# kcat/openal-soft

Hardware: NVIDIA H100
Metric: voice-samples/s mixed (HRTF, bsinc24, 1024-frame updates) (higher is better)
Workload: dtype f32

## Files before the change

openal-soft_b200/csrc/async_ptx.cuh:

```cuda
#pragma once
#include <cstdint>
#include <cuda_runtime.h>

namespace b200mix {

__device__ __forceinline__ uint32_t smem_u32(const void *p)
{ return static_cast<uint32_t>(__cvta_generic_to_shared(p)); }

__device__ __forceinline__ void mbar_init(uint64_t *bar, uint32_t count)
{ asm volatile("mbarrier.init.shared::cta.b64 [%0], %1;" :: "r"(smem_u32(bar)), "r"(count) : "memory"); }
__device__ __forceinline__ void mbar_fence_init()
{ asm volatile("fence.mbarrier_init.release.cluster;" ::: "memory"); }
__device__ __forceinline__ void mbar_expect_tx(uint64_t *bar, uint32_t bytes)
{ asm volatile("mbarrier.arrive.expect_tx.shared::cta.b64 _, [%0], %1;" :: "r"(smem_u32(bar)), "r"(bytes) : "memory"); }
__device__ __forceinline__ void mbar_arrive(uint64_t *bar)
{ asm volatile("mbarrier.arrive.shared::cta.b64 _, [%0];" :: "r"(smem_u32(bar)) : "memory"); }
__device__ __forceinline__ bool mbar_try_wait(uint64_t *bar, uint32_t parity)
{
    uint32_t ok;
    asm volatile("{\n\t.reg .pred p;\n\t"
                 "mbarrier.try_wait.parity.shared::cta.b64 p, [%1], %2;\n\t"
                 "selp.u32 %0, 1, 0, p;\n\t}"
                 : "=r"(ok) : "r"(smem_u32(bar)), "r"(parity) : "memory");
    return ok != 0u;
}
__device__ __forceinline__ void mbar_wait(uint64_t *bar, uint32_t parity)
{ while(!mbar_try_wait(bar, parity)) { } }

__device__ __forceinline__ void bulk_g2s(void *dst_smem, const void *src_gmem, uint32_t bytes, uint64_t *bar)
{
    asm volatile("cp.async.bulk.shared::cluster.global.mbarrier::complete_tx::bytes [%0], [%1], %2, [%3];"
        :: "r"(smem_u32(dst_smem)), "l"(src_gmem), "r"(bytes), "r"(smem_u32(bar)) : "memory");
}
__device__ __forceinline__ void fence_proxy_async_smem()
{ asm volatile("fence.proxy.async.shared::cta;" ::: "memory"); }

__device__ __forceinline__ uint64_t wgmma_smem_desc(uint32_t saddr, uint32_t lbo_bytes, uint32_t sbo_bytes)
{
    return uint64_t((saddr >> 4) & 0x3fffu) | (uint64_t((lbo_bytes >> 4) & 0x3fffu) << 16)
        | (uint64_t((sbo_bytes >> 4) & 0x3fffu) << 32);
}
__device__ __forceinline__ void wgmma_fence() { asm volatile("wgmma.fence.sync.aligned;" ::: "memory"); }
__device__ __forceinline__ void wgmma_commit() { asm volatile("wgmma.commit_group.sync.aligned;" ::: "memory"); }
template<int N> __device__ __forceinline__ void wgmma_wait()
{ asm volatile("wgmma.wait_group.sync.aligned %0;" :: "n"(N) : "memory"); }
__device__ __forceinline__ void wgmma_m64n16k8_tf32(float (&d)[8], uint64_t adesc, uint64_t bdesc, bool accumulate)
{
    asm volatile("{\n\t.reg .pred p;\n\tsetp.ne.b32 p, %10, 0;\n\t"
                 "wgmma.mma_async.sync.aligned.m64n16k8.f32.tf32.tf32 "
                 "{%0,%1,%2,%3,%4,%5,%6,%7}, %8, %9, p, 1, 1;\n\t}"
        : "+f"(d[0]), "+f"(d[1]), "+f"(d[2]), "+f"(d[3]), "+f"(d[4]), "+f"(d[5]), "+f"(d[6]), "+f"(d[7])
        : "l"(adesc), "l"(bdesc), "r"(uint32_t(accumulate)) : "memory");
}

}
```

openal-soft_b200/csrc/b200mix.cu:

```cuda
#include "../../include/b200mix.h"

#include <algorithm>
#include <cmath>
#include <cstdio>
#include <cstdlib>
#include <cstring>
#include <new>
#include <string>
#include <vector>

#include <cuda_runtime.h>

#include <dlfcn.h>

#include "mixer_kernels.cuh"
#include "effect_kernels.cuh"
#include "shard_kernels.cuh"
#include "panmix_tc.cuh"
#include "param_kernels.hpp"
#include "efx_kernels.hpp"
#include "resampler_tables.hpp"
#include "hrtf_store.hpp"
#include "adpcm.hpp"

// ... 119 lines not shown
    bool reverb_upmix{false};
    bool mid_render{false}; uint32_t mid_frames{0};
    bool real_overwrite{false};
    std::vector<uint8_t> h_hrtf;
    std::vector<SendEntry> h_dry_entries;
    SendEntry *d_dry_entries{nullptr};
    uint32_t *d_dry_slot_start{nullptr};
    uint32_t num_dry_entries{0};
    bool dry_entries_dirty{true};
    float *d_dry_partial{nullptr};
    float *d_dry_geff{nullptr};
    float *d_send_geff{nullptr};
    float4 *d_dry_gramp{nullptr}, *d_send_gramp{nullptr};
    float *d_send_partial{nullptr};
    uint32_t send_partial_chunks{0}, max_slot_entries{0};
    bool profile{false};
    cudaEvent_t ev_mix0{nullptr}, ev_mix1{nullptr};
    bool ev_valid{false};
    static constexpr int kStages = 8;
    cudaEvent_t ev_stage[kStages + 1]{};
    bool stage_valid{false}; int profile_level{0};

    std::vector<uint8_t> h_active;
    std::vector<uint32_t> h_cost;
    std::vector<uint32_t> h_order;
    uint32_t *d_order{nullptr};
    uint32_t num_order{0};
    bool order_dirty{true};

    char *h_src{nullptr}, *d_src{nullptr}; uint32_t src_cap{0};
    cudaEvent_t src_done{nullptr}; bool src_busy{false};
    bool dev_filters{false};
    bool panmix_tc{false};

    struct Shard {
        uint32_t rank{0}, world{1}; int transport{0};
        char *own{nullptr}; size_t bytes{0};
        char *peer[kShardMaxWorld]{};
        size_t off_real{0}, off_wet{0}, real_floats{0}, wet_src_floats{0};
        uint32_t owned_max{0};
        uint32_t epoch{0};
        uint32_t *d_counters{nullptr};
        uint32_t *h_status{nullptr};
        cudaEvent_t ev[4]{};
        bool ev_wet{false}, ev_real{false};
        void *nccl_lib{nullptr}; void *comm{nullptr};
        int (*reduce)(const void*, void*, size_t, int, int, int, void*, cudaStream_t){nullptr};
        int (*allreduce)(const void*, void*, size_t, int, int, void*, cudaStream_t){nullptr};
        int (*comm_destroy)(void*){nullptr};
    } shard;

    uint32_t ir_pad{0};
    uint32_t voice_hi{0};
    void (*mix_fn)(const MixParams){nullptr};
    size_t mix_smem{0}; int mix_cdr{0}; int mix_blocks_per_sm{1};
    uint32_t reverb_seq{0};
    uint32_t *d_claim{nullptr};
    int fir_blocks_per_sm{0};
};

namespace {

#define CUDA_TRY(dev, expr) do { cudaError_t e_ = (expr); if(e_ != cudaSuccess) {            \
    (dev)->error = std::string(#expr) + ": " + cudaGetErrorString(e_); return B200MIX_ERR_CUDA; } } while(0)

template<typename T>
int dev_alloc(b200mix_device *d, T *&p, size_t count, bool zero = true)
{
    p = nullptr;
    if(count == 0) return B200MIX_OK;
    CUDA_TRY(d, cudaMalloc(reinterpret_cast<void**>(&p), count*sizeof(T)));
    if(zero) CUDA_TRY(d, cudaMemsetAsync(p, 0, count*sizeof(T), d->stream));
    return B200MIX_OK;
}

using MixKernel = void(*)(const MixParams);

struct FirVariant { MixKernel fn; size_t smem; };
FirVariant get_fir(uint32_t ir_size)
{
    if(ir_size <= 64u)
        return FirVariant{k_hrtf_fir<17, 64>, sizeof(FirSmem<kFirGS, 17, 64>)*kFirGroups};
    return FirVariant{k_hrtf_fir<19, 128>, sizeof(FirSmem<kFirGS, 19, 128>)*kFirGroups};
}

constexpr uint32_t kDryChunksMax = 128;

int ensure_dry_park(b200mix_device *d)
{
    const b200mix_device_desc &dd = d->desc;
    if(d->d_dry_entries) return B200MIX_OK;
    if(!d->d_xscratch)
        if(int rc = dev_alloc(d, d->d_xscratch, size_t(dd.max_voices)*kLine)) return rc;
    if(!d->d_sendinfo)
        if(int rc = dev_alloc(d, d->d_sendinfo, dd.max_voices)) return rc;
    if(int rc = dev_alloc(d, d->d_dry_entries, dd.max_voices)) return rc;
    if(dd.dry_channels > 4u && dd.dry_channels <= uint32_t(kPmN))
    {
        CUDA_TRY(d, cudaFuncSetAttribute(k_panmix_tc, cudaFuncAttributeMaxDynamicSharedMemorySize,
            kPmStages*kPmStageBytes + 1024));
        const char *simt = std::getenv("B200MIX_PANMIX_SIMT");
        d->panmix_tc = !(simt && simt[0] == '1');
    }
    if(int rc = dev_alloc(d, d->d_dry_slot_start, 2)) return rc;
    if(int rc = dev_alloc(d, d->d_dry_partial, size_t(kDryChunksMax)*dd.dry_channels*kLine)) return rc;
    if(int rc = dev_alloc(d, d->d_dry_geff, size_t(dd.max_voices)*dd.dry_channels)) return rc;
    if(int rc = dev_alloc(d, d->d_dry_gramp, size_t(dd.max_voices)*dd.dry_channels)) return rc;
    return B200MIX_OK;
}

static size_t align16(size_t v) { return (v + 15u) & ~size_t(15); }

int ensure_stage(b200mix_device *d, uint32_t n)
{
    if(n <= d->stage_cap) return B200MIX_OK;
    const b200mix_device_desc &dd = d->desc;
    if(d->stage_cap)
    {
        cudaStreamSynchronize(d->stream);
        cudaFreeHost(d->h_arena); cudaFree(d->d_arena);
        d->h_arena = nullptr; d->d_arena = nullptr;
    }
    const uint32_t cap = std::max<uint32_t>(n, 256u);
    const size_t bytes = align16(size_t(cap)*sizeof(VoiceUpdate))
        + align16(size_t(cap)*std::max<size_t>(size_t(dd.ir_size)*2, 4)*sizeof(float))
        + align16(size_t(cap)*dd.dry_channels*sizeof(float))
        + align16(size_t(cap)*dd.num_sends*dd.wet_channels*sizeof(float)) + 64;
    CUDA_TRY(d, cudaMallocHost(reinterpret_cast<void**>(&d->h_arena), bytes));
    CUDA_TRY(d, cudaMalloc(reinterpret_cast<void**>(&d->d_arena), bytes));
    d->h_upd = reinterpret_cast<VoiceUpdate*>(d->h_arena);
    d->stage_cap = cap;
    return B200MIX_OK;
}

const BsincTable *bsinc_for(const b200mix_device *d, uint32_t resampler)
{
    if(resampler < B200MIX_RESAMPLER_FAST_BSINC12 || resampler > B200MIX_RESAMPLER_BSINC48)
        return nullptr;
    return &d->bsinc[(resampler - B200MIX_RESAMPLER_FAST_BSINC12) >> 1];
}

}

extern "C" {

static void shard_release(b200mix_device *d);
static int ensure_filters(b200mix_device *d);

uint32_t b200mix_version(void) { return (1u<<16) | 1u; }

const char *b200mix_last_error(const b200mix_device *dev)
{ return dev ? dev->error.c_str() : g_create_error.c_str(); }

int b200mix_create(const b200mix_device_desc *desc, b200mix_device **out)
{
    if(!desc || !out || desc->struct_size != sizeof(b200mix_device_desc))
    { g_create_error = "bad descriptor"; return B200MIX_ERR_INVALID; }
    if(desc->dry_channels > B200MIX_MAX_DRY_CHANNELS || desc->wet_channels > B200MIX_MAX_WET_CHANNELS
        || desc->num_sends > B200MIX_MAX_SENDS || desc->ir_size > B200MIX_HRIR_LENGTH
        || desc->real_channels > B200MIX_MAX_DRY_CHANNELS || desc->max_voices == 0)
    { g_create_error = "descriptor out of range"; return B200MIX_ERR_INVALID; }
    if((desc->post_process == B200MIX_POST_UHJ && desc->dry_channels < 3)
        || (desc->post_process == B200MIX_POST_TSME && desc->dry_channels < 4))
    { g_create_error = "UHJ post-process needs W,X,Y dry channels"; return B200MIX_ERR_INVALID; }
    if((desc->post_process == B200MIX_POST_HRTF || desc->post_process == B200MIX_POST_UHJ
        || desc->post_process == B200MIX_POST_TSME)
// ... 1365 lines not shown
        std::stable_sort(d->h_order.begin(), d->h_order.end(),
            [d](uint32_t a, uint32_t b) { return d->h_cost[a] > d->h_cost[b]; });
        d->num_order = uint32_t(d->h_order.size());
        if(d->num_order)
        {
            CUDA_TRY(d, cudaMemcpyAsync(d->d_order, d->h_order.data(), d->num_order*sizeof(uint32_t),
                cudaMemcpyHostToDevice, d->stream));
            CUDA_TRY(d, cudaStreamSynchronize(d->stream));
        }
        d->order_dirty = false;
        d->order2_dirty = true;
        d->dry_entries_dirty = true;
    }
    if(d->d_filt && d->order2_dirty)
    {
        d->h_order2.clear();
        for(uint32_t v : d->h_order) if(d->dev_filters || d->h_dfilt[v]) d->h_order2.push_back(v);
        d->num_order2 = uint32_t(d->h_order2.size());
        if(d->num_order2)
        {
            CUDA_TRY(d, cudaMemcpyAsync(d->d_order2, d->h_order2.data(), d->num_order2*sizeof(uint32_t),
                cudaMemcpyHostToDevice, d->stream));
            CUDA_TRY(d, cudaStreamSynchronize(d->stream));
        }
        d->order2_dirty = false;
    }
    const bool hrtfDev = dd.ir_size > 0;
    const uint32_t nv = std::max(d->voice_hi, 1u);
    const uint32_t maxBlocks = uint32_t(d->num_sms*d->mix_blocks_per_sm);
    const uint32_t blocks = std::max(1u, std::min(maxBlocks, (d->num_order + kMixGroups - 1)/kMixGroups));

    MixParams P{};
    P.voices = d->d_voices; P.buffers = d->d_buffers;
    P.hrtf_tgt = d->d_hrtf_tgt; P.hrtf_old = d->d_hrtf_old;
    P.dry_cur = d->d_dry_cur; P.dry_tgt = d->d_dry_tgt;
    P.partial = d->d_partial;
    P.results = want_results ? d->d_results : nullptr;
    for(int i = 0;i < 3;++i) P.bsinc_tab[i] = d->d_bsinc[i];
    for(int i = 0;i < 2;++i) P.cubic_tab[i] = d->d_cubic[i];
    P.max_voices = nv; P.frames = frames; P.ir_pad = d->ir_pad;
    P.cd = dd.dry_channels; P.num_sends = dd.num_sends;
    P.order = d->d_order; P.num_order = d->num_order;
    P.xscratch = d->d_xscratch; P.sendinfo = d->d_sendinfo;
    P.filt = d->d_filt; P.filt_paths = 1u + dd.num_sends;
    P.qhdr = d->d_qhdr; P.queue = d->d_queue;
    P.claim = d->d_claim;
    P.dline = d->d_dline;
    stage_mark(d, 1);
    if(d->profile) cudaEventRecord(d->ev_mix0, d->stream);
    d->mix_fn<<<blocks, kMixGS*kMixGroups, d->mix_smem, d->stream>>>(P);
    ++d->launches;
    CUDA_TRY(d, cudaGetLastError());

    stage_mark(d, 2);
    size_t rows2 = 0;
    if(d->d_filt && d->num_order2)
    {
        FilterRunParams FP{};
        FP.filt = d->d_filt; FP.filt_paths = 1u + dd.num_sends; FP.sendinfo = d->d_sendinfo;
        FP.direct_order = d->d_order2; FP.num_direct = d->num_order2;
        FP.xscratch = d->d_xscratch; FP.dline = d->d_dline; FP.frames = frames;
        k_filters<<<(d->num_order2 + 31u)/32u, 32, 0, d->stream>>>(FP);
        ++d->launches;
        if(d->mix_cdr > 0)
        {
            const uint32_t blocks2 = std::max(1u, std::min(maxBlocks, (d->num_order2 + kMixGroups - 1)/kMixGroups));
            rows2 = blocks2;
            MixParams P2 = P;
            P2.order = d->d_order2; P2.num_order = d->num_order2;
            P2.partial = d->d_partial + d->partial_floats;
            P2.results = nullptr;
            k_mix_deferred<kMixGS, kMixGroups, 4><<<blocks2, kMixGS*kMixGroups,
                sizeof(DeferredSmem<kMixGroups, 4>), d->stream>>>(P2);
            ++d->launches;
        }
        CUDA_TRY(d, cudaGetLastError());
    }
    uint32_t firBlocks = 0;
    if(hrtfDev)
    {
        const FirVariant fir = get_fir(dd.ir_size);
        firBlocks = std::max(1u, std::min(uint32_t(d->num_sms*d->fir_blocks_per_sm),
            (d->num_order + kFirGroups - 1)/kFirGroups));
        fir.fn<<<firBlocks, kFirGS*kFirGroups, fir.smem, d->stream>>>(P);
        ++d->launches;
        CUDA_TRY(d, cudaGetLastError());
    }
    if(d->profile) { cudaEventRecord(d->ev_mix1, d->stream); d->ev_valid = true; }

    stage_mark(d, 3);
    if(hrtfDev)
    {
        const uint32_t len = 2*kAccumLen;
        k_reduce_rows<<<(len/4 + kReduceCols - 1)/kReduceCols, 1024, 0, d->stream>>>(d->d_partial, firBlocks, len,
            d->d_accum_sum, 0);
        ++d->launches;
    }
    if(d->mix_cdr > 0)
    {
        const uint32_t len = uint32_t(d->mix_cdr)*kLine;
        k_reduce_rows<<<(len/4 + kReduceCols - 1)/kReduceCols, 1024, 0, d->stream>>>(d->d_partial, blocks, len, d->d_dry, 1);
        ++d->launches;
        if(rows2)
        {
            k_reduce_rows<<<(len/4 + kReduceCols - 1)/kReduceCols, 1024, 0, d->stream>>>(d->d_partial + d->partial_floats,
                uint32_t(rows2), len, d->d_dry, 1);
            ++d->launches;
        }
    }
    CUDA_TRY(d, cudaGetLastError());

    stage_mark(d, 4);
    if(d->mix_cdr == 0 && d->d_dry_entries)
    {
        if(d->dry_entries_dirty)
        {
            d->h_dry_entries.clear();
            for(uint32_t v = 0;v < d->voice_hi;++v)
                if(d->h_active[v] && !d->h_hrtf[v]) d->h_dry_entries.push_back(SendEntry{v, 0u});
            d->num_dry_entries = uint32_t(d->h_dry_entries.size());
            const uint32_t ss[2] = {0u, d->num_dry_entries};
            CUDA_TRY(d, cudaMemcpyAsync(d->d_dry_slot_start, ss, sizeof(ss), cudaMemcpyHostToDevice, d->stream));
            if(d->num_dry_entries)
                CUDA_TRY(d, cudaMemcpyAsync(d->d_dry_entries, d->h_dry_entries.data(),
                    d->num_dry_entries*sizeof(SendEntry), cudaMemcpyHostToDevice, d->stream));
            CUDA_TRY(d, cudaStreamSynchronize(d->stream));
            d->dry_entries_dirty = false;
        }
        if(d->num_dry_entries)
        {
            SendMixParams DM{};
            DM.slot_start = d->d_dry_slot_start; DM.entries = d->d_dry_entries; DM.sendinfo = d->d_sendinfo;
            DM.xscratch = d->d_xscratch; DM.send_cur = d->d_dry_cur; DM.send_tgt = d->d_dry_tgt;
            DM.wet = d->d_dry; DM.frames = frames; DM.cw = dd.dry_channels; DM.num_sends = 1;
            DM.valid_bit = kSiDry; DM.dline = d->d_dline ? d->d_dline : d->d_xscratch;
            const uint32_t chunks = std::max(1u, std::min(kDryChunksMax, (d->num_dry_entries + 63u)/64u));
            DM.chunks = chunks; DM.partial = d->d_dry_partial; DM.geff = d->d_dry_geff; DM.gramp = d->d_dry_gramp;
            const bool tc = d->panmix_tc && dd.dry_channels > 4u && dd.dry_channels <= uint32_t(kPmN)
                && frames == uint32_t(kLine) && chunks > 1u;
            if(int rc = run_bus_mix(d, DM, d->num_dry_entries, 1u, tc)) return rc;
        }
    }

    stage_mark(d, 5);
    if((d->active_slots || force_sends) && d->d_wet && d->d_slot_start)
    {
        if(d->sends_dirty)
        {
            d->h_slot_start.assign(dd.max_slots + 1, 0);
            d->h_entries.clear();
            for(uint32_t sl = 0;sl < dd.max_slots;++sl)
            {
                d->h_slot_start[sl] = uint32_t(d->h_entries.size());
                for(uint32_t v = 0;v < d->voice_hi;++v)
                    for(uint32_t s2 = 0;s2 < dd.num_sends;++s2)
                        if(d->h_send_slot[size_t(v)*B200MIX_MAX_SENDS + s2] == sl)
                            d->h_entries.push_back(SendEntry{v, s2});
            }
            d->h_slot_start[dd.max_slots] = uint32_t(d->h_entries.size());
            d->num_entries = uint32_t(d->h_entries.size());
            d->max_slot_entries = 0;
            for(uint32_t sl = 0;sl < dd.max_slots;++sl)
                d->max_slot_entries = std::max(d->max_slot_entries, d->h_slot_start[sl+1] - d->h_slot_start[sl]);
            CUDA_TRY(d, cudaMemcpyAsync(d->d_slot_start, d->h_slot_start.data(),
                (dd.max_slots + 1)*sizeof(uint32_t), cudaMemcpyHostToDevice, d->stream));
            if(d->num_entries)
                CUDA_TRY(d, cudaMemcpyAsync(d->d_entries, d->h_entries.data(),
                    d->num_entries*sizeof(SendEntry), cudaMemcpyHostToDevice, d->stream));
            CUDA_TRY(d, cudaStreamSynchronize(d->stream));
            d->sends_dirty = false;
        }
        SendMixParams SM{};
        SM.slot_start = d->d_slot_start; SM.entries = d->d_entries; SM.sendinfo = d->d_sendinfo;
        SM.xscratch = d->d_xscratch; SM.send_cur = d->d_send_cur; SM.send_tgt = d->d_send_tgt;
        SM.wet = d->d_wet; SM.frames = frames; SM.cw = dd.wet_channels; SM.num_sends = dd.num_sends;
        SM.valid_bit = kSiSend;
        if(d->d_filt && d->num_entries)
        {
// ... 75 lines not shown
                        mask |= 1u << old;
                    }
                }
                R.offset += frames;
                if(d->h_slots[sl].rv_mask != mask || d->h_slots[sl].rv_cur != uint32_t(R.cur))
                {
                    d->h_slots[sl].rv_mask = mask; d->h_slots[sl].rv_cur = uint32_t(R.cur);
                    CUDA_TRY(d, cudaMemcpyAsync(d->d_slots + sl, &d->h_slots[sl], sizeof(SlotRec),
                        cudaMemcpyHostToDevice, d->stream));
                    CUDA_TRY(d, cudaStreamSynchronize(d->stream));
                }
            }
        }
        SlotMixParams SP{};
        SP.slots = d->d_slots; SP.dry = d->d_dry; SP.frames = frames; SP.cd = dd.dry_channels;
        SP.num_slots = dd.max_slots; SP.wet = d->d_wet; SP.cw = dd.wet_channels;
        for(uint32_t st = 0;st < d->num_stages;++st)
        {
            if(d->reverb_slots)
            {
                ReverbParamsK RP{};
                RP.slots = d->d_slots; RP.wet = d->d_wet; RP.cubic = d->d_cubic_filter;
                RP.frames = frames; RP.cw = dd.wet_channels; RP.stage = st;
                RP.seq = ++d->reverb_seq;
                k_reverb_process<<<dim3(dd.max_slots, 2, 2), 128, 0, d->stream>>>(RP);
                k_reverb_commit<<<dd.max_slots, 2, 0, d->stream>>>(RP);
                d->launches += 2;
                if(d->reverb_upmix)
                {
                    k_reverb_upmix<<<dim3(dd.max_slots, 2), 256, 8*kLine*sizeof(float), d->stream>>>(RP);
                    ++d->launches;
                }
            }
            CP.stage = st; SP.stage = st;
            if(d->efx_slots)
            {
                EfxRunParams EQ{d->d_efx_views, d->d_wet, frames, dd.wet_channels, st, d->d_cubic_filter};
                CUDA_TRY(d, launch_efx_process(EQ, dd.max_slots, d->stream));
                ++d->launches;
                if(d->pshift_slots)
                {
                    CUDA_TRY(d, launch_efx_pshift(EQ, dd.max_slots, d->stream));
                    ++d->launches;
                }
            }
            if(convWork)
            {
                k_conv_input<<<dd.max_slots, 128, 0, d->stream>>>(CP);
                k_conv_mac<<<dim3(dd.max_slots, convCh, CP.chunks), 128, sizeof(ConvMacSmem), d->stream>>>(CP);
                k_conv_ifft<<<dim3(dd.max_slots, convCh, kConvMaxBlocks), 128, 0, d->stream>>>(CP);
                k_conv_output<<<dim3(dd.max_slots, convCh), 128, 0, d->stream>>>(CP);
                d->launches += 4;
            }
            k_slot_output_mix<<<dim3((frames + 127)/128, dd.dry_channels), 128, 0, d->stream>>>(SP);
            ++d->launches;
            if(d->any_target)
            {
                k_slot_target_mix<<<dim3((frames + 127)/128, dd.max_slots), 128, 0, d->stream>>>(SP);
                ++d->launches;
            }
        }
        k_slot_gains_commit<<<dd.max_slots, 64, 0, d->stream>>>(SP);
        ++d->launches;
        for(auto &eh : d->efx)
        {
            if(eh.used && eh.p.type == B200MIX_EFFECT_MODULATOR) eh.mod_index = (eh.mod_index + frames) % eh.mod_range;
            if(eh.used && eh.p.type == B200MIX_EFFECT_CHORUS) eh.lfo_offset = (eh.lfo_offset + frames) % eh.lfo_range;
        }
        CUDA_TRY(d, cudaGetLastError());
    }

    stage_mark(d, 7);
    switch(dd.post_process)
    {
    case B200MIX_POST_HRTF:
    {
        PostHrtfParams Q{};
        Q.accum_sum = d->d_accum_sum; Q.carry_in = d->d_carry[d->carry_idx];
        Q.carry_out = d->d_carry[d->carry_idx^1];
        Q.dry = d->d_dry; Q.real = d->d_real; Q.dec_coef = d->d_dec_coef;
        Q.dec_hfscale = d->d_dec_hfscale; Q.dec_state = d->d_dec_state; Q.temp = d->d_temp;
        Q.frames = frames; Q.cd = dd.dry_channels; Q.dec_ir = d->dec_ir;
        Q.real_left = dd.real_left; Q.real_right = dd.real_right; Q.dry_active = d->dry_active;
        if(d->dry_active)
        {
            k_post_hrtf_split<<<dd.dry_channels, 32, 0, d->stream>>>(Q);
            ++d->launches;
        }
        Q.overwrite = d->real_overwrite ? 1u : 0u;
        k_post_hrtf_mix<<<dim3((frames + kHrirLen + 127)/128, 2), 128, 0, d->stream>>>(Q);
        ++d->launches;
        d->carry_idx ^= 1;
        break;
    }
    case B200MIX_POST_AMBIDEC:
    {
        PostAmbiParams Q{};
        Q.dry = d->d_dry; Q.real = d->d_real; Q.gains_hf = d->d_amb_hf; Q.gains_lf = d->d_amb_lf;
        Q.split_state = d->d_amb_state; Q.temp_hf = d->d_temp; Q.temp_lf = d->d_temp2;
        Q.frames = frames; Q.cd = dd.dry_channels; Q.real_channels = dd.real_channels;
        Q.dual = d->amb_dual;
        if(d->amb_dual)
        {
            k_post_ambi_split<<<1, 32, 0, d->stream>>>(Q);
            ++d->launches;
        }
        const uint32_t total = dd.real_channels*frames;
        k_post_ambi_mix<<<(total + 127)/128, 128, 0, d->stream>>>(Q);
        ++d->launches;
        if(d->stab_center != B200MIX_NO_SLOT)
        {
            StabParams S{};
            S.real = d->d_real; S.state = d->d_stab_state; S.frames = frames;
            S.real_channels = dd.real_channels; S.lidx = dd.real_left; S.ridx = dd.real_right;
            S.cidx = d->stab_center; S.coeff = d->stab_coeff;
            const float halfPi = 3.14159265358979323846f*0.5f;
            S.mid_lf = std::cos(1.0f/3.0f * halfPi); S.mid_hf = std::cos(1.0f/4.0f * halfPi);
            S.center_lf = std::sin(1.0f/3.0f * halfPi); S.center_hf = std::sin(1.0f/4.0f * halfPi);
            const size_t smem = size_t(2u + dd.real_channels)*kLine*sizeof(float);
            k_post_stabilizer<<<1, 32u*dd.real_channels, smem, d->stream>>>(S);
            ++d->launches;
        }
        else if(d->bs2b_level)
        {
            Bs2bParams B{d->d_real, d->d_bs2b, d->d_bs2b + 4, frames, dd.real_left, dd.real_right};
            k_post_bs2b<<<1, 128, 0, d->stream>>>(B);
            ++d->launches;
        }
        break;
    }
    case B200MIX_POST_UHJ: case B200MIX_POST_TSME:
    {
        const MatrixEncSpec spec = dd.post_process == B200MIX_POST_TSME ? kTsmeEncSpec : kUhjEncSpec;
        PostUhjParams Q{};
        Q.dry = d->d_dry; Q.real = d->d_real; Q.state = d->d_uhj_state; Q.scratch = d->d_uhj_scratch;
        Q.frames = frames; Q.real_left = dd.real_left; Q.real_right = dd.real_right; Q.enc = spec;
        if(d->uhj_fir)
        {
            PostUhjFirParams F{d->d_dry, d->d_real, d->d_uhj_fir_state, d->d_uhj_fir_coef, frames,
                dd.real_left, dd.real_right, d->uhj_fir, spec};
            k_post_uhj_fir<<<1, 1024, 0, d->stream>>>(F);
        }
        else
            k_post_uhj<<<1, 1024, 0, d->stream>>>(Q);
        ++d->launches;
        break;
    }
    default: break;
    }
    stage_mark(d, 8);
    if(d->profile_level >= 2) d->stage_valid = true;
    CUDA_TRY(d, cudaGetLastError());
    return B200MIX_OK;
}

static int render_output_stage(b200mix_device *d, uint32_t frames)
{
    const b200mix_device_desc &dd = d->desc;
    if(d->shard.transport && d->shard.rank != 0u) return B200MIX_OK;
    if(d->d_limiter)
    {
        LimiterParams LQ{d->d_limiter, d->d_real, d->d_limiter_delay, frames};
        k_limiter<<<1, 1024, 0, d->stream>>>(LQ);
        ++d->launches;
    }
    if(d->d_dc_delay)
    {
        DistCompParams DQ{d->d_real, d->d_dc_buf, d->d_dc_delay, d->d_dc_gain, frames};
        k_distance_comp<<<dd.real_channels, 1024, 0, d->stream>>>(DQ);
        ++d->launches;
    }
    CUDA_TRY(d, cudaGetLastError());
    return B200MIX_OK;
// ... 604 lines not shown
```

openal-soft_b200/csrc/mixer_kernels.cuh:

```cuda
#pragma once
#include <cstddef>
#include <cstdint>
#include <cuda_runtime.h>

#include "voice_structs.hpp"
#include "async_ptx.cuh"

namespace b200mix {

constexpr int kLine = 1024;
constexpr int kHrirLen = 128;
constexpr int kHist = 64;
constexpr int kEdge = 24;
constexpr int kPad = 48;
constexpr int kResBuf = kLine + 256 + kPad;
constexpr int kSrcSizeMax = kResBuf - kEdge;
constexpr int kAccumLen = kLine + kHrirLen;
constexpr float kSilence = 0.00001f;
constexpr float kEps = 1.1920929e-07f;

constexpr uint32_t kVfStatic = 1u<<2, kVfLooping = 1u<<3, kVfHrtf = 1u<<4;
constexpr uint32_t kVfFading = 1u<<8, kVfHaveBuffer = 1u<<9, kVfCoefDirty = 1u<<10;
constexpr uint32_t kUpNoBuffer = 1u<<11;
constexpr uint32_t kVfChannelMask = 0xffu<<16;
// ... 942 lines not shown
            looping = false;
        const uint32_t resampler = h0.w;
        const bool isQueue = !(flags & kVfStatic) && P.qhdr != nullptr;
        const uint4 qh = isQueue ? P.qhdr[v] : make_uint4(0u, 0u, kNoLoop, 0u);
        const uint32_t *qitems = P.queue + size_t(v)*kMaxQueue;
        const bool isHrtf = CDR == 0 && P.ir_pad != 0u && (flags & kVfHrtf);
        const bool dirty = (flags & kVfCoefDirty) != 0;
        FilterRec *dfilt = P.filt ? P.filt + size_t(v)*P.filt_paths : nullptr;
        const bool defer = dfilt && dfilt->active;
        const bool playing = vstate == 1u;

        for(int k = t;k < kPad;k += GS) S.win[k] = rec.prev[k];
        uint32_t m, tapOff, ms;
        build_phase_table<GS>(P, S.tabF, S.tabD, resampler, increment, h2, h3, t, m, tapOff, ms);
        float *xs = CDR > 0 ? S.x : P.xscratch + size_t(v)*kLine;
        if(CDR == 0) prefetch_next_voices<GS>(P, oi, groups, t);

        for(uint32_t loaded = 0;loaded < n;)
        {
            uint32_t dstn, srcn;
            calc_buffer_size(fracPos, increment, n-loaded, dstn, srcn);
            uint32_t srcDelay = 0;
            bool silent = false;
            bool packedWin = false;
            if(dstn == 0u) { dstn = n - loaded; silent = true; }
            if(intPos < 0)
            {
                srcDelay = uint32_t(-intPos);
                if(srcDelay >= srcn) silent = true;
            }
            group_sync(bar, GS);
            if(silent)
            {
                for(uint32_t k = t;k < dstn;k += GS) xs[loaded+k] = 0.0f;
                for(uint32_t k = t;k < srcn;k += GS) S.win[kEdge+k] = 0.0f;
            }
            else
            {
                float *srcBuffer = S.win + kEdge;
                bool winInt = false;
                const bool pack = resampler >= 4u && !(increment == 65536u && fracPos == 0u);
                if(!haveBuffer) hold_end_sample<GS>(srcBuffer, srcn, t, bar);
                else
                {
                    const uint32_t uintPos = intPos < 0 ? 0u : uint32_t(intPos);
                    const uint32_t count = srcn - srcDelay;
                    for(uint32_t k = t;k < srcDelay;k += GS) srcBuffer[k] = 0.0f;
                    winInt = stage_span_tma<GS>(S.win, &S.tmaBar, tmaPhase, buf, flags, isQueue, looping,
                            loopStart, loopEnd, uintPos, srcDelay, count, pack, packedWin, t, bar)
                        || gather_span<GS>(P, buf, flags, isQueue, qh, qitems, looping, loopStart, loopEnd,
                            uintPos, count, srcBuffer + srcDelay, t, bar);
                }
                group_sync(bar, GS);

                if(pack && winInt && !packedWin)
                {
                    pack_window16<GS>(S.win, srcn, t, bar);
                    packedWin = true;
                }
                resample_chunk<GS>(S.win, S.tabF, S.tabD, xs, loaded, dstn, increment, fracPos,
                    resampler, m, tapOff, ms, packedWin, t);
            }
            advance_chunk<GS>(S.win, rec.prev, packedWin, silent, playing, n, loaded, dstn, increment,
                fracPos, intPos, t, bar);
        }
        group_sync(bar, GS);

        const uint32_t counter = (flags & kVfFading) ? (n < 64u ? n : 64u) : 0u;
        if(P.sendinfo)
            park_voice<GS, CDR>(P, xs, v, rec.send_mask, defer, isHrtf, playing, dirty, counter, t);
        if(dfilt && !defer) filter_clear(*dfilt, t);
        if constexpr(CDR > 0)
            if(!defer)
                mix_dry<GS, CDR>(accD, xs, S.newGain, P.dry_cur + size_t(v)*P.cd, P.dry_tgt + size_t(v)*P.cd,
                    P.cd, n, counter, playing, t);
        if(t == 0)
            write_back_voice(P, rec, v, h1, flags, vstate, increment, haveBuffer, isQueue, qh, qitems,
                looping, loopStart, loopEnd, buf.frames);
        group_sync(bar, GS);
        if(CDR > 0 && !defer) store_dry_gains(P.dry_cur + size_t(v)*P.cd, S.newGain, P.cd, t);
        group_sync(bar, GS);
    }

    if constexpr(CDR > 0) store_partial_row<GS, GROUPS, CDR>(accD, smem_raw, P.partial, g, t);
}

template<int GROUPS, int CDR>
union DeferredSmem {
    struct { float x[kLine]; float newGain[32]; } group[GROUPS];
    float stage[CDR*kLine];
};

template<int GS, int GROUPS, int CDR>
__global__ void __launch_bounds__(GS*GROUPS)
k_mix_deferred(const MixParams P)
{
    extern __shared__ __align__(16) unsigned char smem_raw[];
    const int g = threadIdx.x / GS;
    const int t = threadIdx.x % GS;
    auto &S = reinterpret_cast<DeferredSmem<GROUPS, CDR>*>(smem_raw)->group[g];
    const int bar = 1 + g;
    constexpr int SPT = kLine / GS;

    float accD[CDR][SPT];
    #pragma unroll
    for(int c = 0;c < CDR;++c)
        #pragma unroll
        for(int r = 0;r < SPT;++r) accD[c][r] = 0.0f;

    const uint32_t n = P.frames;
    const uint32_t groups = gridDim.x*GROUPS;
    for(uint32_t oi = blockIdx.x*GROUPS + g;oi < P.num_order;oi += groups)
    {
        const uint32_t v = P.order[oi];
        const uint32_t info = P.sendinfo[v];
        if(!(info & kSiDeferred)) continue;
        const float *fl = P.dline + size_t(v)*kLine;
        for(uint32_t k = t;k < n;k += GS) S.x[k] = fl[k];
        group_sync(bar, GS);
        mix_dry<GS, CDR>(accD, S.x, S.newGain, P.dry_cur + size_t(v)*P.cd, P.dry_tgt + size_t(v)*P.cd,
            P.cd, n, (info >> 8) & 0xffu, (info & kSiPlaying) != 0, t);
        group_sync(bar, GS);
        store_dry_gains(P.dry_cur + size_t(v)*P.cd, S.newGain, P.cd, t);
    }

    store_partial_row<GS, GROUPS, CDR>(accD, smem_raw, P.partial, g, t);
}

constexpr int kFirGS = 64, kFirGroups = 2, kFirCtasPerSm = 4;

__device__ __forceinline__ uint32_t next_hrtf_voice(const MixParams &P, uint32_t oi, uint32_t stride,
    uint32_t &v, uint32_t &info)
{
    for(;oi < P.num_order;oi += stride)
    {
        v = P.order[oi];
        info = P.sendinfo[v];
        if(info & kSiHrtf) break;
    }
    return oi;
}

__device__ __forceinline__ void fir_stage_issue(const MixParams &P, FirStage &B, uint64_t *bar,
    uint32_t v, uint32_t info, uint32_t n)
{
    const uint32_t lineBytes = (n & ~3u)*4u, irBytes = P.ir_pad*8u;
    const bool dirty = (info & kSiDirty) != 0;
    const float *line = ((info & kSiDeferred) ? P.dline : P.xscratch) + size_t(v)*kLine;
    fence_proxy_async_smem();
    mbar_expect_tx(bar, kHist*4u + lineBytes + (dirty ? 2u : 1u)*irBytes);
    bulk_g2s(B.x, P.voices[v].hist, kHist*4u, bar);
    if(lineBytes) bulk_g2s(B.x + kHist, line, lineBytes, bar);
    bulk_g2s(B.coefT, P.hrtf_tgt + size_t(v)*P.ir_pad, irBytes, bar);
    if(dirty) bulk_g2s(B.coefO, P.hrtf_old + size_t(v)*P.ir_pad, irBytes, bar);
}

template<int OPT, int FP>
__global__ void __launch_bounds__(kFirGS*kFirGroups, kFirCtasPerSm)
k_hrtf_fir(const MixParams P)
{
    constexpr int GS = kFirGS, GROUPS = kFirGroups;
    using Smem = FirSmem<GS, OPT, FP>;
    extern __shared__ __align__(16) unsigned char smem_raw[];
    const int g = threadIdx.x / GS;
    const int t = threadIdx.x % GS;
    Smem &S = reinterpret_cast<Smem*>(smem_raw)[g];
    const int bar = 1 + g;
    const int t0 = OPT*t;
    const uint32_t n = P.frames;

    float2 acc[OPT];
    #pragma unroll
    for(int r = 0;r < OPT;++r) acc[r] = make_float2(0.0f, 0.0f);

    for(int i = t;i < FP;i += GS) S.lLR[i] = make_float2(0.0f, 0.0f);
    for(int i = FP + int(n) + t;i < Smem::kLLen;i += GS) S.lLR[i] = make_float2(0.0f, 0.0f);
    if(t == 0) { mbar_init(&S.bar[0], 1u); mbar_init(&S.bar[1], 1u); mbar_fence_init(); }
    group_sync(bar, GS);

    const uint32_t stride = gridDim.x*GROUPS;
    uint32_t v = 0u, info = 0u;
    uint32_t oi = next_hrtf_voice(P, blockIdx.x*GROUPS + g, stride, v, info);
    if(t == 0 && oi < P.num_order) fir_stage_issue(P, S.st[0], &S.bar[0], v, info, n);
    uint32_t parity = 0u;
    for(int b = 0;oi < P.num_order;b ^= 1)
    {
        VoiceRec &rec = P.voices[v];
        const uint4 *hp = reinterpret_cast<const uint4*>(&rec);
        const uint4 h3 = hp[3], h4 = hp[4];

        uint32_t vN = 0u, infoN = 0u;
        const uint32_t oiN = next_hrtf_voice(P, oi + stride, stride, vN, infoN);
        if(t == 0 && oiN < P.num_order) fir_stage_issue(P, S.st[b^1], &S.bar[b^1], vN, infoN, n);

        FirStage &B = S.st[b];
        const bool playing = (info & kSiPlaying) != 0;
        const bool dirty = (info & kSiDirty) != 0;
        const uint32_t counter = (info >> 8) & 0xffu;

        const float *line = ((info & kSiDeferred) ? P.dline : P.xscratch) + size_t(v)*kLine;
        for(uint32_t k = (n & ~3u) + t;k < n;k += GS) B.x[kHist + k] = line[k];
        mbar_wait(&S.bar[b], (parity >> b) & 1u);
        parity ^= 1u << b;
        if(n & 3u) group_sync(bar, GS);

        if(playing)
            for(int k = t;k < kHist;k += GS) rec.hist[k] = B.x[n + k];
        uint32_t oD0 = h4.x, oD1 = h4.y;
        float oGain = __uint_as_float(h4.z);
        const uint32_t tD0 = h3.y, tD1 = h3.z;
        const float tgtGain = __uint_as_float(h3.w);
        if(!counter) { oD0 = tD0; oD1 = tD1; oGain = tgtGain; }
        const bool sameFilter = !counter || (!dirty && oD0 == tD0 && oD1 == tD1);
        const float targetGain = tgtGain * (playing ? 1.0f : 0.0f);
        const uint32_t fademix = counter;
        float blendNewStep = 0.0f, oldStep = 0.0f;
        bool oldOn = false, newOn = false;
        float gainA = oGain;
        if(fademix)
        {
            const float gain = targetGain;
            blendNewStep = gain / float(fademix);
            oldStep = oGain / float(fademix);
            oldOn = oGain > kSilence;
            newOn = blendNewStep*float(fademix) > kSilence;
            gainA = gain;
        }
        const uint32_t todo = n - fademix;
        const float step2 = todo ? (targetGain - gainA) / float(todo) : 0.0f;

        const float *hs = B.x;
        float2 *in = S.lLR + FP;
        for(uint32_t s = t;s < fademix;s += GS)
        {
            const float gnew = (newOn && s >= 1u) ? blendNewStep*float(s) : 0.0f;
            float l = hs[kHist - tD0 + s] * gnew;
            float r = hs[kHist - tD1 + s] * gnew;
            if(sameFilter && oldOn)
            {
                const float gold = oldStep*float(fademix - s);
                l += hs[kHist - oD0 + s] * gold;
                r += hs[kHist - oD1 + s] * gold;
            }
            in[s] = make_float2(l, r);
        }
        const float *xl = hs + kHist - tD0, *xr = hs + kHist - tD1;
        for(uint32_t s = fademix + t;s < n;s += GS)
        {
            const float gnew = gainA + step2*float(s - fademix);
            in[s] = make_float2(xl[s] * gnew, xr[s] * gnew);
        }
        const bool oldPass = !sameFilter && oldOn;
        if(oldPass)
            for(int i = t;i < Smem::kOLen;i += GS)
            {
                const int s = i - FP;
                float l = 0.0f, r = 0.0f;
                if(s >= 0 && uint32_t(s) < fademix)
                {
                    const float gold = oldStep*float(fademix - uint32_t(s));
                    l = hs[kHist - oD0 + s] * gold;
                    r = hs[kHist - oD1 + s] * gold;
                }
                S.oLR[i] = make_float2(l, r);
            }
        group_sync(bar, GS);

        const int irpad = int(P.ir_pad);
        fir_pass<OPT, FP>(acc, S.lLR, B.coefT, irpad, t0);
        if(oldPass && t0 < int(kHist) + irpad)
            fir_pass<OPT, FP>(acc, S.oLR, dirty ? B.coefO : B.coefT, irpad, t0);
        if(t == 0)
        {
            rec.old_delay0 = tD0; rec.old_delay1 = tD1;
            rec.old_gain = targetGain;
        }
        group_sync(bar, GS);
        oi = oiN; v = vN; info = infoN;
    }

    const size_t row = blockIdx.x;
    __syncthreads();
    float *stage = reinterpret_cast<float*>(smem_raw);
    for(int gg = 0;gg < GROUPS;++gg)
    {
        if(g == gg)
        {
            #pragma unroll
            for(int r = 0;r < OPT;++r)
            {
                const int o = t0 + r;
                if(o < kAccumLen)
                {
                    if(gg == 0) { stage[o] = acc[r].x; stage[kAccumLen + o] = acc[r].y; }
                    else { stage[o] += acc[r].x; stage[kAccumLen + o] += acc[r].y; }
                }
            }
            if(gg == 0 && GS*OPT < kAccumLen)
                for(int o = GS*OPT + t;o < kAccumLen;o += GS) { stage[o] = 0.0f; stage[kAccumLen + o] = 0.0f; }
        }
        __syncthreads();
    }
    float *pl = P.partial + row*(2*kAccumLen);
    for(int o = threadIdx.x;o < 2*kAccumLen;o += GS*GROUPS) pl[o] = stage[o];
}


constexpr int kReduceCols = 8, kReduceSegs = 128;
__global__ void __launch_bounds__(1024)
k_reduce_rows(const float *__restrict__ partial, uint32_t rows, uint32_t len,
    float *__restrict__ out, int accumulate)
{
    __shared__ float4 sm[kReduceSegs][kReduceCols];
    const uint32_t col = threadIdx.x & (kReduceCols-1), seg = threadIdx.x / kReduceCols;
    const uint32_t e4 = blockIdx.x*kReduceCols + col;
    float4 s = make_float4(0.f, 0.f, 0.f, 0.f);
    if(e4*4u < len)
    {
        const uint32_t per = (rows + kReduceSegs - 1u)/kReduceSegs;
        const uint32_t r0 = seg*per, r1 = (r0 + per < rows) ? r0 + per : rows;
        const float4 *p = reinterpret_cast<const float4*>(partial) + e4;
        const size_t stride4 = len/4u;
        uint32_t r = r0;
        for(;r + 4u <= r1;r += 4u)
        {
            const float4 a = __ldg(p + size_t(r)*stride4), b = __ldg(p + size_t(r+1)*stride4);
            const float4 c = __ldg(p + size_t(r+2)*stride4), d = __ldg(p + size_t(r+3)*stride4);
            s.x += a.x; s.y += a.y; s.z += a.z; s.w += a.w;
            s.x += b.x; s.y += b.y; s.z += b.z; s.w += b.w;
            s.x += c.x; s.y += c.y; s.z += c.z; s.w += c.w;
            s.x += d.x; s.y += d.y; s.z += d.z; s.w += d.w;
        }
        for(;r < r1;++r)
        {
            const float4 a = __ldg(p + size_t(r)*stride4);
            s.x += a.x; s.y += a.y; s.z += a.z; s.w += a.w;
        }
    }
    sm[seg][col] = s;
    __syncthreads();
    #pragma unroll
    for(uint32_t width = kReduceSegs/4u;width >= 1u;width /= 4u)
    {
        float4 tot = make_float4(0.f, 0.f, 0.f, 0.f);
        const bool on = seg < width;
        if(on)
        {
            tot = sm[seg*4u][col];
            #pragma unroll
            for(uint32_t k = 1;k < 4u;++k)
            {
                const float4 a = sm[seg*4u + k][col];
                tot.x += a.x; tot.y += a.y; tot.z += a.z; tot.w += a.w;
            }
        }
        __syncthreads();
        if(on) sm[seg][col] = tot;
        __syncthreads();
        if(width == 2u) break;
    }
    if(seg == 0 && e4*4u < len)
    {
        float4 tot = sm[0][col];
        const float4 b = sm[1][col];
        tot.x += b.x; tot.y += b.y; tot.z += b.z; tot.w += b.w;
        float4 *o = reinterpret_cast<float4*>(out) + e4;
        if(accumulate)
        {
            const float4 a = *o;
            tot.x += a.x; tot.y += a.y; tot.z += a.z; tot.w += a.w;
        }
        *o = tot;
    }
}

__global__ void __launch_bounds__(256)
k_reduce_few(const float *__restrict__ partial, uint32_t rows, uint32_t len,
    float *__restrict__ out, int accumulate)
{
    const uint32_t e4 = blockIdx.x*blockDim.x + threadIdx.x;
    if(e4*4u >= len) return;
    const float4 *p = reinterpret_cast<const float4*>(partial) + e4;
    const size_t stride4 = len/4u;
    float4 v[16];
    #pragma unroll
    for(uint32_t r = 0;r < 16u;++r)
        v[r] = r < rows ? __ldg(p + size_t(r)*stride4) : make_float4(0.f, 0.f, 0.f, 0.f);
    float4 g[4];
    #pragma unroll
    for(uint32_t j = 0;j < 4u;++j)
    {
        float4 t = v[4u*j];
        #pragma unroll
        for(uint32_t k = 1;k < 4u;++k)
        { t.x += v[4u*j+k].x; t.y += v[4u*j+k].y; t.z += v[4u*j+k].z; t.w += v[4u*j+k].w; }
        g[j] = t;
// ... 183 lines not shown
        const float *src = fromDirs ? nullptr : A.coeffs + size_t(u)*A.ir*2;
        for(uint32_t k = t;k < A.ir_pad;k += 64)
        {
            if(!wasDirty && !reset) ol[k] = tg[k];
            float2 val = make_float2(0.f, 0.f);
            if(fromDirs)
            {
                if(k < A.st_ir && k < A.ir)
                {
                    val = (k == 0) ? make_float2(sB.passthru, sB.passthru) : val;
                    #pragma unroll
                    for(int c = 0;c < 4;++c)
                    {
                        const float2 sv = A.st_coeffs[size_t(sB.idx[c])*A.st_ir + k];
                        val.x = __fadd_rn(__fmul_rn(sv.x, sB.w[c]), val.x);
                        val.y = __fadd_rn(__fmul_rn(sv.y, sB.w[c]), val.y);
                    }
                }
            }
            else if(k < A.ir) val = make_float2(src[k*2], src[k*2+1]);
            tg[k] = val;
        }
    }
    if(up.has_dry && A.dry_tgt)
        for(uint32_t c = t;c < A.cd;c += 64)
            A.dry_tgt[size_t(up.voice)*A.cd + c] = A.dry[size_t(u)*A.cd + c];
    if(A.send && A.send_tgt)
        for(uint32_t c = t;c < A.num_sends*A.cw;c += 64)
            A.send_tgt[size_t(up.voice)*A.num_sends*A.cw + c] = A.send[size_t(u)*A.num_sends*A.cw + c];
    if(t == 0)
    {
        uint32_t fl = up.flags & (kVfStatic|kVfLooping|kVfHrtf|kVfChannelMask);
        if(reset)
        {
            rec.pos = up.position; rec.frac = up.position_frac;
            fl |= kVfHaveBuffer;
            if(up.flags & (1u<<6)) fl |= kVfFading;
            rec.old_delay0 = 0; rec.old_delay1 = 0; rec.old_gain = 0.0f;
            if(A.qhdr) A.qhdr[up.voice].y = 0u;
        }
        else
        {
            fl |= oldFlags & (kVfFading|kVfHaveBuffer|kVfCoefDirty);
        }
        if(up.has_coeffs && !reset) fl |= kVfCoefDirty;
        if(up.flags & kUpNoBuffer) fl &= ~kVfHaveBuffer;
        rec.flags = fl;
        if(up.flags & (1u<<7)) rec.state = 0u;
        else if(up.flags & (1u<<1)) rec.state = 2u;
        else if(up.flags & (1u<<0)) rec.state = 1u;
        rec.buffer = up.buffer; rec.resampler = up.resampler;
        rec.loop_start = up.loop_start; rec.loop_end = up.loop_end; rec.step = up.step;
        rec.bsinc_sf = up.bsinc_sf; rec.bsinc_m = up.bsinc_m; rec.bsinc_l = up.bsinc_l;
        rec.bsinc_off = up.bsinc_off;
        rec.tgt_delay0 = fromDirs ? sB.delay[0] : up.delay0;
        rec.tgt_delay1 = fromDirs ? sB.delay[1] : up.delay1;
        rec.tgt_gain = up.gain;
        uint32_t mask = 0;
        for(int s = 0;s < kMaxSends;++s)
        {
            rec.send_slot[s] = up.send_slot[s];
            if(up.send_slot[s] != 0xffffffffu) mask |= 1u<<s;
        }
        rec.send_mask = mask;
    }
}

struct PostHrtfParams {
    const float *accum_sum;
    const float *carry_in;
    float *carry_out;
    const float *dry;
    float *real;
    const float2 *dec_coef;
    const float *dec_hfscale; float *dec_state;
    float *temp;
    uint32_t frames, cd, dec_ir, real_left, real_right, dry_active;
    uint32_t overwrite;
};

__global__ void __launch_bounds__(32) k_post_hrtf_split(const PostHrtfParams Q)
{
    __shared__ float line[kLine];
    const uint32_t c = blockIdx.x;
    if(c >= Q.cd) return;
    const uint32_t lane = threadIdx.x, n = Q.frames;
    const float *in = Q.dry + size_t(c)*kLine;
    float *out = Q.temp + size_t(c)*kLine;
    for(uint32_t i = lane;i < kLine;i += 32) line[i] = (i < n) ? in[i] : 0.0f;
    __syncwarp();
    if(lane == 0)
    {
        float *st = Q.dec_state + c*4;
        const float ap_coeff = st[0];
        const float lp_coeff = st[0]*0.5f + 0.5f;
        float lp_z1 = st[1], lp_z2 = st[2], ap_z1 = st[3];
        const float hfscale = Q.dec_hfscale[c];
        for(uint32_t i0 = 0;i0 < n;i0 += 8)
        {
            float x[8], y[8];
            #pragma unroll
            for(int k = 0;k < 8;++k) x[k] = line[i0+k];
            #pragma unroll
            for(int k = 0;k < 8;++k)
            {
                const float d0 = (x[k] - lp_z1) * lp_coeff;
                const float lp_y0 = lp_z1 + d0;
                const float nz1 = lp_y0 + d0*lp_coeff;
                const float d1 = (lp_y0 - lp_z2) * lp_coeff;
                const float lp_y1 = lp_z2 + d1;
                const float nz2 = lp_y1 + d1;
                const float ap_y = x[k]*ap_coeff + ap_z1;
                const float naz = x[k] - ap_y*ap_coeff;
                y[k] = (ap_y-lp_y1)*hfscale + lp_y1;
                if(i0 + k < n) { lp_z1 = nz1; lp_z2 = nz2; ap_z1 = naz; }
            }
            #pragma unroll
            for(int k = 0;k < 8;++k) line[i0+k] = y[k];
        }
        st[1] = lp_z1; st[2] = lp_z2; st[3] = ap_z1;
    }
    __syncwarp();
    for(uint32_t i = lane;i < n;i += 32) out[i] = line[i];
}

__global__ void __launch_bounds__(128) k_post_hrtf_mix(const PostHrtfParams Q)
{
    __shared__ float xs[128 + kHrirLen];
    __shared__ float cf[kHrirLen];
    const uint32_t span = Q.frames + kHrirLen;
    const uint32_t ear = blockIdx.y;
    const uint32_t t0 = blockIdx.x*128u, tt = t0 + threadIdx.x;
    float tot = 0.0f;
    if(tt < span)
    {
        tot = Q.accum_sum[ear*kAccumLen + tt];
        if(tt < uint32_t(kHrirLen)) tot += Q.carry_in[ear*kHrirLen + tt];
    }
    if(Q.dry_active)
    {
        const uint32_t jmax = Q.dec_ir;
        for(uint32_t c = 0;c < Q.cd;++c)
        {
            const float *x = Q.temp + size_t(c)*kLine;
            const float2 *cg = Q.dec_coef + size_t(c)*Q.dec_ir;
            __syncthreads();
            for(uint32_t k = threadIdx.x;k < 128u + kHrirLen;k += 128u)
            {
                const int src = int(t0) - int(kHrirLen) + int(k);
                xs[k] = (src >= 0 && src < int(Q.frames)) ? x[src] : 0.0f;
            }
            if(threadIdx.x < jmax) cf[threadIdx.x] = ear ? cg[threadIdx.x].y : cg[threadIdx.x].x;
            __syncthreads();
            float s = 0.0f;
            const float *w = xs + kHrirLen + threadIdx.x;
            for(uint32_t j = 0;j < jmax;++j)
                s = fmaf(cf[j], w[-int(j)], s);
            tot += s;
        }
    }
    if(tt >= span) return;
    if(tt < Q.frames)
    {
        float *o = Q.real + size_t(ear ? Q.real_right : Q.real_left)*kLine + tt;
        *o = Q.overwrite ? tot : (*o + tot);
    }
    else
        Q.carry_out[ear*kHrirLen + (tt - Q.frames)] = tot;
}

struct PostAmbiParams {
    const float *dry; float *real; const float *gains_hf; const float *gains_lf;
    float *split_state; float *temp_hf; float *temp_lf;
    uint32_t frames, cd, real_channels, dual;
};

__global__ void k_post_ambi_split(const PostAmbiParams Q)
{
    const uint32_t c = blockIdx.x*blockDim.x + threadIdx.x;
    if(c >= Q.cd) return;
    float *st = Q.split_state + c*4;
    const float ap_coeff = st[0];
    const float lp_coeff = st[0]*0.5f + 0.5f;
    float lp_z1 = st[1], lp_z2 = st[2], ap_z1 = st[3];
    const float *in = Q.dry + size_t(c)*kLine;
    float *hp = Q.temp_hf + size_t(c)*kLine, *lp = Q.temp_lf + size_t(c)*kLine;
    for(uint32_t i = 0;i < Q.frames;++i)
    {
        const float x = in[i];
        const float d0 = (x - lp_z1) * lp_coeff;
        const float lp_y0 = lp_z1 + d0;
        lp_z1 = lp_y0 + d0;
        const float d1 = (lp_y0 - lp_z2) * lp_coeff;
        const float lp_y1 = lp_z2 + d1;
        lp_z2 = lp_y1 + d1;
        lp[i] = lp_y1;
        const float ap_y = x*ap_coeff + ap_z1;
        ap_z1 = x - ap_y*ap_coeff;
        hp[i] = ap_y - lp_y1;
    }
    st[1] = lp_z1; st[2] = lp_z2; st[3] = ap_z1;
}

__global__ void __launch_bounds__(128) k_post_ambi_mix(const PostAmbiParams Q)
{
    const uint32_t idx = blockIdx.x*blockDim.x + threadIdx.x;
    if(idx >= Q.real_channels*Q.frames) return;
    const uint32_t o = idx / Q.frames, i = idx - o*Q.frames;
    float acc = Q.real[size_t(o)*kLine + i];
    for(uint32_t c = 0;c < Q.cd;++c)
    {
        if(Q.dual)
        {
// ... 662 lines not shown
```

Before: 31.01 billion.

## Use programmatic dependent launch for FIR, reduce, and post-HRTF kernels

```diff
diff --git a/openal-soft_b200/csrc/async_ptx.cuh b/openal-soft_b200/csrc/async_ptx.cuh
--- a/openal-soft_b200/csrc/async_ptx.cuh
+++ b/openal-soft_b200/csrc/async_ptx.cuh
@@ -35,6 +35,10 @@
 __device__ __forceinline__ void fence_proxy_async_smem()
 { asm volatile("fence.proxy.async.shared::cta;" ::: "memory"); }
 
+__device__ __forceinline__ void griddep_wait() { asm volatile("griddepcontrol.wait;" ::: "memory"); }
+__device__ __forceinline__ void griddep_launch_dependents()
+{ asm volatile("griddepcontrol.launch_dependents;" ::: "memory"); }
+
 __device__ __forceinline__ uint64_t wgmma_smem_desc(uint32_t saddr, uint32_t lbo_bytes, uint32_t sbo_bytes)
 {
     return uint64_t((saddr >> 4) & 0x3fffu) | (uint64_t((lbo_bytes >> 4) & 0x3fffu) << 16)
diff --git a/openal-soft_b200/csrc/b200mix.cu b/openal-soft_b200/csrc/b200mix.cu
--- a/openal-soft_b200/csrc/b200mix.cu
+++ b/openal-soft_b200/csrc/b200mix.cu
@@ -225,6 +225,19 @@
     if(ir_size <= 64u)
         return FirVariant{k_hrtf_fir<17, 64>, sizeof(FirSmem<kFirGS, 17, 64>)*kFirGroups};
     return FirVariant{k_hrtf_fir<19, 128>, sizeof(FirSmem<kFirGS, 19, 128>)*kFirGroups};
+}
+
+template<typename... Args>
+cudaError_t launch(const b200mix_device *d, bool pdl, void (*fn)(Args...), dim3 grid, dim3 block, size_t smem,
+    Args... args)
+{
+    cudaLaunchAttribute attr{};
+    attr.id = cudaLaunchAttributeProgrammaticStreamSerialization;
+    attr.val.programmaticStreamSerializationAllowed = 1;
+    cudaLaunchConfig_t cfg{};
+    cfg.gridDim = grid; cfg.blockDim = block; cfg.dynamicSmemBytes = smem; cfg.stream = d->stream;
+    cfg.attrs = &attr; cfg.numAttrs = pdl ? 1u : 0u;
+    return cudaLaunchKernelEx(&cfg, fn, args...);
 }
 
 constexpr uint32_t kDryChunksMax = 128;
@@ -1756,7 +1769,7 @@
         const FirVariant fir = get_fir(dd.ir_size);
         firBlocks = std::max(1u, std::min(uint32_t(d->num_sms*d->fir_blocks_per_sm),
             (d->num_order + kFirGroups - 1)/kFirGroups));
-        fir.fn<<<firBlocks, kFirGS*kFirGroups, fir.smem, d->stream>>>(P);
+        CUDA_TRY(d, launch(d, d->profile_level < 2, fir.fn, dim3(firBlocks), dim3(kFirGS*kFirGroups), fir.smem, P));
         ++d->launches;
         CUDA_TRY(d, cudaGetLastError());
     }
@@ -1766,8 +1779,8 @@
     if(hrtfDev)
     {
         const uint32_t len = 2*kAccumLen;
-        k_reduce_rows<<<(len/4 + kReduceCols - 1)/kReduceCols, 1024, 0, d->stream>>>(d->d_partial, firBlocks, len,
-            d->d_accum_sum, 0);
+        CUDA_TRY(d, launch(d, d->profile_level < 2, k_reduce_rows, dim3((len/4 + kReduceCols - 1)/kReduceCols),
+            dim3(1024), 0, static_cast<const float*>(d->d_partial), firBlocks, len, d->d_accum_sum, 0));
         ++d->launches;
     }
     if(d->mix_cdr > 0)
@@ -2009,13 +2022,14 @@
         Q.dec_hfscale = d->d_dec_hfscale; Q.dec_state = d->d_dec_state; Q.temp = d->d_temp;
         Q.frames = frames; Q.cd = dd.dry_channels; Q.dec_ir = d->dec_ir;
         Q.real_left = dd.real_left; Q.real_right = dd.real_right; Q.dry_active = d->dry_active;
+        const bool pdl = d->profile_level < 2;
         if(d->dry_active)
         {
-            k_post_hrtf_split<<<dd.dry_channels, 32, 0, d->stream>>>(Q);
+            CUDA_TRY(d, launch(d, pdl, k_post_hrtf_split, dim3(dd.dry_channels), dim3(32), 0, Q));
             ++d->launches;
         }
         Q.overwrite = d->real_overwrite ? 1u : 0u;
-        k_post_hrtf_mix<<<dim3((frames + kHrirLen + 127)/128, 2), 128, 0, d->stream>>>(Q);
+        CUDA_TRY(d, launch(d, pdl, k_post_hrtf_mix, dim3((frames + kHrirLen + 127)/128, 2), dim3(128), 0, Q));
         ++d->launches;
         d->carry_idx ^= 1;
         break;
diff --git a/openal-soft_b200/csrc/mixer_kernels.cuh b/openal-soft_b200/csrc/mixer_kernels.cuh
--- a/openal-soft_b200/csrc/mixer_kernels.cuh
+++ b/openal-soft_b200/csrc/mixer_kernels.cuh
@@ -1048,6 +1048,7 @@
         group_sync(bar, GS);
     }
 
+    if constexpr(CDR == 0) griddep_launch_dependents();
     if constexpr(CDR > 0) store_partial_row<GS, GROUPS, CDR>(accD, smem_raw, P.partial, g, t);
 }
 
@@ -1142,9 +1143,17 @@
     for(int i = t;i < FP;i += GS) S.lLR[i] = make_float2(0.0f, 0.0f);
     for(int i = FP + int(n) + t;i < Smem::kLLen;i += GS) S.lLR[i] = make_float2(0.0f, 0.0f);
     if(t == 0) { mbar_init(&S.bar[0], 1u); mbar_init(&S.bar[1], 1u); mbar_fence_init(); }
+    const uint32_t stride = gridDim.x*GROUPS;
+    for(uint32_t k = 0, oiK = blockIdx.x*GROUPS + g;k < 2u && oiK < P.num_order;++k, oiK += stride)
+    {
+        const uint32_t vK = P.order[oiK];
+        const char *ir = reinterpret_cast<const char*>(P.hrtf_tgt + size_t(vK)*P.ir_pad);
+        for(uint32_t a = uint32_t(t)*128u;a < P.ir_pad*8u;a += GS*128u) prefetch_l2(ir + a);
+        if(t < kHist/32) prefetch_l2(P.voices[vK].hist + 32*t);
+    }
+    griddep_wait();
     group_sync(bar, GS);
 
-    const uint32_t stride = gridDim.x*GROUPS;
     uint32_t v = 0u, info = 0u;
     uint32_t oi = next_hrtf_voice(P, blockIdx.x*GROUPS + g, stride, v, info);
     if(t == 0 && oi < P.num_order) fir_stage_issue(P, S.st[0], &S.bar[0], v, info, n);
@@ -1278,6 +1287,7 @@
     float *__restrict__ out, int accumulate)
 {
     __shared__ float4 sm[kReduceSegs][kReduceCols];
+    griddep_wait();
     const uint32_t col = threadIdx.x & (kReduceCols-1), seg = threadIdx.x / kReduceCols;
     const uint32_t e4 = blockIdx.x*kReduceCols + col;
     float4 s = make_float4(0.f, 0.f, 0.f, 0.f);
@@ -1627,6 +1637,7 @@
 __global__ void __launch_bounds__(32) k_post_hrtf_split(const PostHrtfParams Q)
 {
     __shared__ float line[kLine];
+    griddep_wait();
     const uint32_t c = blockIdx.x;
     if(c >= Q.cd) return;
     const uint32_t lane = threadIdx.x, n = Q.frames;
@@ -1674,6 +1685,7 @@
     __shared__ float xs[128 + kHrirLen];
     __shared__ float cf[kHrirLen];
     const uint32_t span = Q.frames + kHrirLen;
+    griddep_wait();
     const uint32_t ear = blockIdx.y;
     const uint32_t t0 = blockIdx.x*128u, tt = t0 + threadIdx.x;
     float tot = 0.0f;
```

After: 31.75 billion, median of 6. 2.4% higher.
